# MoonLab-YH/AOD_MEH_HUA

Hardware: AMD Instinct MI355X
Metric: images/sec train+HUA-score, RetinaNet-R50 VOC 512^2 (higher is better)
Workload: dtype bf16x3

## Files before the change

### aod_meh_hua_amd/_C.py

```python
import ctypes as C
import os

import torch

_HERE = os.path.dirname(os.path.abspath(__file__))
LIB_PATH = os.environ.get('AOD_HIP_LIB') or os.path.join(_HERE, 'lib', 'libaodhip.so')


class AodHipError(RuntimeError):
    pass


if not os.path.exists(LIB_PATH):
    raise ImportError(f'{LIB_PATH} is missing: run `python -m aod_meh_hua_amd.build` (hipcc, gfx950). '
                      'There is no CPU fallback for the MEH/HUA hot path.')
lib = C.CDLL(LIB_PATH)


class ConvSeg(C.Structure):
    _fields_ = [('B', C.c_int32), ('H', C.c_int32), ('W', C.c_int32), ('OH', C.c_int32), ('OW', C.c_int32),
                ('src_row0', C.c_int64), ('dst_row0', C.c_int64)]


class ConvDesc(C.Structure):
# ... 22 lines not shown
    'aod_bottleneck128x3_fwd': (C.c_int, [P, I32, I32, I32, P, P, P, P, P, P, P, P, P, P, P, P, P]),
    'aod_bottleneck128_fwd': (C.c_int, [P, I32, I32, I32, P, P, P, P, P, P, P, P, P, P, P, P, P]),
    'aod_frag_pack': (C.c_int, [P, I32, I32, P]),
    'aod_frag_pack_item_bytes': (C.c_int, []),
    'aod_bottleneck256f_fwd': (C.c_int, [P, I32, I32, I32, P, P, P, P, P, P, P, P, P, P, P, P, P]),
    'aod_bottleneck256f_bwd': (C.c_int, [P, I32, I32, I32, P, P, P, P, P, P, P, P, P, P, P, P, P]),
    'aod_bottleneck_bwd': (C.c_int, [I32, P, I32, I32, I32, P, P, P, P, P, P, P, P, P, P, P, P, P]),
    'aod_bottleneck256_fwd': (C.c_int, [P, I32, I32, I32, P, P, P, P, P, P, P, P, P, P, P, P, P]),
    'aod_conv2d': (C.c_int, [C.POINTER(ConvDesc), P, P, P, P, P, P, P, P, P, P, P]),
    'aod_conv2d_ws_bytes': (SZ, [C.POINTER(ConvDesc)]),
    'aod_conv2d_ws': (C.c_int, [C.POINTER(ConvDesc), P, P, P, P, P, P, P, P, P, P, P, SZ, P]),
    'aod_conv2d_plan': (C.c_int, [C.POINTER(ConvDesc), I32, C.c_uint, C.POINTER(ConvPlan)]),
    'aod_conv2d_grouped': (C.c_int, [C.POINTER(ConvDesc), I32, P, P, P, P, P, P, P]),
    'aod_conv2d_ws_map': (C.c_int, [C.POINTER(ConvDesc), P, P, P, P, P, P, P, P, P, P, P, SZ, P, P, P]),
    'aod_conv2d_grouped_map': (C.c_int, [C.POINTER(ConvDesc), I32, P, P, P, P, P, P, P, P, P]),
    'aod_halo_conv3x3_applies': (C.c_int, [C.POINTER(ConvDesc)]),
    'aod_halo_conv3x3': (C.c_int, [C.POINTER(ConvDesc), P, P, P, P, P, P, P]),
    'aod_conv2d_wgrad': (C.c_int, [C.POINTER(ConvDesc), P, P, P, P, P]),
    'aod_conv2d_wgrad_splits': (C.c_int, [C.POINTER(ConvDesc)]),
    'aod_conv2d_wgrad_slabs': (C.c_int, [C.POINTER(ConvDesc), P, P, P, I32, I64, P, P]),
    'aod_conv2d_wgrad_slabs_map': (C.c_int, [C.POINTER(ConvDesc), P, P, P, I32, I64, P, P, P]),
    'aod_conv2d_wgrad_group_plan': (C.c_int, [P, I32, P]),
    'aod_conv2d_wgrad_grouped': (C.c_int, [P, I32, P, P, P, P, P, P, P]),
    'aod_conv2d_wgrad_plan': (C.c_int, [P, I32, P, P, P]),
    'aod_conv2d_wgrad_grouped_map': (C.c_int, [P, I32, P, P, P, P, P, P, P, P]),
    'aod_unpack_wgrad_slabs_grouped': (C.c_int, [I32, P, P, P, P, P, P, P, P, P, P, P, P, P, P, P, P, P]),
    'aod_unpack_wgrad_slabs': (C.c_int, [P, I32, I64, P, I32, I32, I32, I32, I32, I32, P, P, P, P, P, P, P]),
    'aod_conv_row_table_bytes': (SZ, [C.POINTER(ConvDesc)]),
    'aod_conv_row_table': (C.c_int, [C.POINTER(ConvDesc), P, P]),
    'aod_pack_weight_fwd': (C.c_int, [P, P, I32, I32, I32, I32, I32, P]),
# ... 124 lines not shown
```

### aod_meh_hua_amd/csrc/conv.hip

```cpp
#include "common.h"
#include "pointwise.h"
#include "conv_x3p.h"

struct ConvGroup { const bf16_t* x; const bf16_t* w; void* y; const float* pre_shift; const bf16_t* mask; float* colsum; const unsigned char* omap; };
struct ConvKParams {
  const bf16_t* x;
  const bf16_t* w;
  void* y;
  const float* pre_scale;
  const float* pre_shift;
  const bf16_t* res;
  const bf16_t* mask;
  const float* post_scale;
  bf16_t* zraw;
  float* colsum;
  int C, N, K, R, S, stride, pad, dil, transposed, relu, out_f32;
  int nseg, M;
  int tiles_m, tiles_n;
  int ksplit;
  float* ws;
  int perm;
  int ngroups;
  int interleave;
  const unsigned char* omap;
// ... 13 lines not shown
#ifdef AOD_TILE_TIMING
__device__ unsigned long long* g_tile_stamps = nullptr;
extern "C" int aod_dbg_set_tile_stamps(void* buf) { return (int)hipMemcpyToSymbol(HIP_SYMBOL(g_tile_stamps), &buf, sizeof(buf)); }
#define TSTAMP(k) do { if (g_tile_stamps && threadIdx.x == 0) g_tile_stamps[(size_t)blockIdx.x * 16 + (k)] = wall_clock64(); } while (0)
#else
#define TSTAMP(k) do {} while (0)
#endif

__device__ __forceinline__ unsigned udiv_small(unsigned n, unsigned d) {
  unsigned q = (unsigned)((float)n * __builtin_amdgcn_rcpf((float)d));
  const int r = (int)(n - q * d);
  q = r < 0 ? q - 1 : ((unsigned)r >= d ? q + 1 : q);
  return q;
}

__device__ __forceinline__ int xcd_swizzle(int bid, int nwg) {
  const int q = nwg >> 3, r = nwg & 7, xcd = bid & 7, j = bid >> 3;
  return (xcd < r ? xcd * (q + 1) : r * (q + 1) + (xcd - r) * q) + j;
}

template <int BM, int BN, int NT, int OPS, bool GROUPED, int ST, bool X3>
__global__ __launch_bounds__(NT) __attribute__((amdgpu_waves_per_eu(BM >= 192 ? 2 : (NT == 512 ? 4 : 1), BM >= 192 ? 2 : (NT == 512 ? 4 : 8)))) void conv_igemm_kernel(const ConvKParams p) {
  static_assert(NT == 256 || NT == 512, "4 or 8 waves");
  static_assert(ST == 2 || (ST == 3 && NT == 256), "LDS stages: 2, or 3 for the 4-wave forms");
  static_assert(!X3 || NT == 256 || (NT == 512 && (BM == 256 || BM == 192 || BM == 128)), "X3: the 4-wave forms, the 8-wave 256 x 256 / 192 x 192 tiles and (A/B) the 8-wave 128 x 128 tile");
  constexpr int BK = 64;
  constexpr int CPR = BK / 8;
  constexpr int RPP = NT / CPR;
  constexpr int A_IT = BM / RPP, B_IT = BN / RPP;
  constexpr int ROWB = BK * 2;
  constexpr int A_BYTES = BM * ROWB, B_BYTES = BN * ROWB, STAGE = A_BYTES + B_BYTES;
  constexpr int WAVES_M = NT / 128;
  constexpr int WM = BM / WAVES_M, WN = BN / 2;
// ... 3 lines not shown
  constexpr int EBM = BM / EP;
  constexpr bool PREFETCH = EP == 1 && !X3;
  extern __shared__ __attribute__((aligned(16))) char smem[];

  const int t = threadIdx.x;
  TSTAMP(0);
  const int lane = t & 63, wave = t >> 6;
  const int wm = wave >> 1, wn = wave & 1;
  const int nwg = p.tiles_m * p.tiles_n;
  int wg;
  if (!p.perm) wg = xcd_swizzle(blockIdx.x, nwg * (GROUPED ? p.ngroups : p.ksplit));
  else if ((nwg & 31) == 0) {
    const int x = blockIdx.x & 7, j = blockIdx.x >> 3, q = j & 3, k = j >> 2, tq = nwg >> 2;
    wg = q * tq + x * (tq >> 3) + k;
  } else wg = blockIdx.x;
  const bool il = GROUPED && p.interleave;
  const int tile = il ? wg / p.ngroups : wg % nwg, zz = il ? wg % p.ngroups : wg / nwg;
  const int kz = GROUPED ? 0 : zz;
  const int gi = GROUPED ? zz : 0;
#define AOD_GSEL(f, dflt) (GROUPED ? (gi == 0 ? p.grp[0].f : (gi == 1 ? p.grp[1].f : (gi == 2 ? p.grp[2].f : p.grp[3].f))) : (dflt))
  const bf16_t* const g_x = AOD_GSEL(x, p.x);
  const bf16_t* const g_w = AOD_GSEL(w, p.w);
  const float* const g_shift = AOD_GSEL(pre_shift, p.pre_shift);
#define g_y AOD_GSEL(y, p.y)
#define g_mask AOD_GSEL(mask, p.mask)
#define g_colsum AOD_GSEL(colsum, p.colsum)
  const int tile_n = tile % p.tiles_n, tile_m = tile / p.tiles_n;
  const int m0 = tile_m * BM, n0 = tile_n * BN;
  if constexpr (X3 && (GROUPED || NT == 256)) {
    const unsigned char* const om = AOD_GSEL(omap, p.omap);
    if (om) {
      const int mend = m0 + BM < p.M ? m0 + BM : p.M;
// ... 839 lines not shown
    const char* ksplit_steps = getenv("AOD_KSPLIT_STEPS");
    const char* stagger = getenv("AOD_STAGGER");
    const char* x3_taps_inner = getenv("AOD_X3_TAPS_INNER");
    const char* dgrad_lattice = getenv("AOD_DGRAD_LATTICE");
    const char* dgrad_classes = getenv("AOD_DGRAD_CLASSES");
    const char* tile_want = getenv("AOD_TILE_WANT");
    const char* tile_256 = getenv("AOD_TILE_256");
    const char* x3_128_w8 = getenv("AOD_X3_128_W8");
    const char* x3_128_st3 = getenv("AOD_X3_128_ST3");
    const char* tile_w8 = getenv("AOD_TILE_W8");
    const char* ring3 = getenv("AOD_RING3");
  };
  static const Once& once() { static const Once k{}; return k; }

  enum Call { X3P_OVER_256, X3_TILE_192, X3P_GROUPED, X3P, X3P_PRE, X3P_BN, X3P_DGRAD, X3P_LATTICE, X3P_MIN_STEPS, X3P_PRE_MIN_STEPS, X3P_MIN_TILES,
              X3P_ROT, SPARSE_BWD, NCALL };
  const char* val[NCALL];
  unsigned seen = 0;
  const char* call(Call k) {
    static const char* const names[NCALL] = {"AOD_X3P_OVER_256", "AOD_X3_TILE_192", "AOD_X3P_GROUPED", "AOD_X3P", "AOD_X3P_PRE", "AOD_X3P_BN",
                                             "AOD_X3P_DGRAD", "AOD_X3P_LATTICE", "AOD_X3P_MIN_STEPS", "AOD_X3P_PRE_MIN_STEPS", "AOD_X3P_MIN_TILES",
                                             "AOD_X3P_ROT", "AOD_SPARSE_BWD"};
    if (!((seen >> k) & 1u)) { val[k] = getenv(names[k]); seen |= 1u << k; }
    return val[k];
  }
  bool is(Call k, char c) { const char* v = call(k); return v && v[0] == c; }
};
static bool knob_is(const char* v, char c) { return v && v[0] == c; }

static int xp_cus() {
  static int cus[64];
  int dev = 0;
  if (hipGetDevice(&dev) != hipSuccess || dev < 0 || dev > 63) return 256;
  if (!cus[dev]) {
    int n = 0;
    if (hipDeviceGetAttribute(&n, hipDeviceAttributeMultiprocessorCount, dev) != hipSuccess || n <= 0) n = 256;
    cus[dev] = n;
// ... 74 lines not shown
                       nullptr, colsum ? colsum[0] : nullptr, p);
  if (rc) return rc;
  AOD_CHECK_ARG(!p.perm, "conv_grouped: class-major stride-2 dgrad launches are not grouped");
  p.ngroups = ngroups;
  for (int g = 0; g < ngroups; ++g) {
    AOD_CHECK_ARG(src[g] && w_packed[g] && dst[g], "conv_grouped: null operand in group %d", g);
    p.grp[g].x = (const bf16_t*)src[g]; p.grp[g].w = (const bf16_t*)w_packed[g]; p.grp[g].y = dst[g];
    p.grp[g].pre_shift = pre_shift ? pre_shift[g] : nullptr;
    p.grp[g].mask = mask ? (const bf16_t*)mask[g] : nullptr;
    p.grp[g].colsum = colsum ? colsum[g] : nullptr;
  }
  return 0;
}

struct MapGeo { int nseg, M, R, S, pad, dil; int segH[8], segW[8], seg_mend[8]; };
__global__ __launch_bounds__(256) void row_map_dilate_kernel(const unsigned char* __restrict__ in, unsigned char* __restrict__ out, const MapGeo g) {
  const int b = (int)(blockIdx.x * 256 + threadIdx.x);
  if (b >= (g.M + 63) >> 6) return;
  const int r0 = b << 6, r1 = r0 + 63 < g.M ? r0 + 63 : g.M - 1;
  const int up = (g.R - 1) * g.dil - g.pad, dn = g.pad, lf = (g.S - 1) * g.dil - g.pad, rt = g.pad;
  int any = 0;
  for (int sg = 0; sg < g.nseg; ++sg) {
    const int s0 = sg ? g.seg_mend[sg - 1] : 0, s1 = g.seg_mend[sg];
    const int lo = (r0 > s0 ? r0 : s0) - s0, hi = (r1 < s1 - 1 ? r1 : s1 - 1) - s0;
    if (lo > hi) continue;
    const int W = g.segW[sg], hw = g.segH[sg] * W;
    int a = lo - up * W - lf, z = hi + dn * W + rt;
    const int qa = (lo / W - up) * W, qz = (hi / W + dn + 1) * W - 1;
    a = a > qa ? a : qa; z = z < qz ? z : qz;
    const int ia = (lo / hw) * hw, iz = (hi / hw + 1) * hw - 1;
    a = a > ia ? a : ia; z = z < iz ? z : iz;
    for (int k = (s0 + a) >> 6; k <= (s0 + z) >> 6; ++k) any |= in[k];
  }
  out[b] = any ? 1 : 0;
}

static int conv_map_setup(ConvKParams& p, int ngroups, const void* const* in_map, void* const* out_map, hipStream_t st) {
  const int ng = ngroups ? ngroups : 1;
  bool any = false;
  for (int g = 0; g < ng; ++g) {
    AOD_CHECK_ARG(!in_map[g] == !out_map[g], "conv (map): member %d needs both its incoming and its outgoing map, or neither", g);
    any = any || in_map[g];
  }
  if (!any || p.M == 0) return 0;
  AOD_CHECK_ARG(p.x3 && p.transposed && p.stride == 1 && !p.out_f32 && !p.perm && !p.up_w, "conv (map): row-activity maps exist for the x3 stride-1 dgrad with X-layout rows only");
  AOD_CHECK_ARG((p.R - 1) * p.dil >= p.pad && (p.S - 1) * p.dil >= p.pad, "conv (map): padding beyond the filter");
  MapGeo mg;
  memset(&mg, 0, sizeof(mg));
  mg.nseg = p.nseg; mg.M = p.M; mg.R = p.R; mg.S = p.S; mg.pad = p.pad; mg.dil = p.dil;
// ... 5 lines not shown
  }
  const int nblk = (p.M + 63) >> 6;
  ConvKnobs kn;
  const bool dense = kn.is(ConvKnobs::SPARSE_BWD, '0');
  for (int g = 0; g < ng; ++g) {
    if (!in_map[g]) continue;
    hipLaunchKernelGGL(row_map_dilate_kernel, dim3((nblk + 255) / 256), dim3(256), 0, st, (const unsigned char*)in_map[g], (unsigned char*)out_map[g], mg);
    AOD_LAUNCH_CHECK();
    const float* const shift = ngroups ? p.grp[g].pre_shift : p.pre_shift;
    float* const cs = ngroups ? p.grp[g].colsum : p.colsum;
    const bool skip_ok = !dense && !shift && !p.pre_scale && !p.res && !p.post_scale && !p.zraw && !(cs && aod_get_deterministic());
    if (!skip_ok) continue;
    if (ngroups) { p.grp[g].omap = (const unsigned char*)out_map[g]; p.interleave = 1; }
    else p.omap = (const unsigned char*)out_map[g];
  }
  return 0;
}

extern "C" size_t aod_conv2d_ws_bytes(const aod_conv_desc_t* desc) {
  ConvKParams p;
  memset(&p, 0, sizeof(p));
  if (!desc || fill_params(desc, p) != 0 || p.M == 0) return 0;
  const int ks = choose_ksplit(p);
  return ks > 1 ? (size_t)ks * p.M * p.N * 4 : 0;
}

static void pw_args(const ConvKParams& p, PwArgs& a) {
  const long long s0 = p.seg_src0[0], d0 = p.seg_dst0[0];
  a.x = p.x + s0 * p.C; a.w = p.w; a.y = reinterpret_cast<bf16_t*>(p.y) + d0 * p.N;
  a.pre_scale = p.pre_scale; a.pre_shift = p.pre_shift;
// ... 238 lines not shown
  if (p.M == 0) return 0;
  rc = conv_plan(p, ngroups, false, pl);
  if (rc) return rc;
  AOD_CHECK_ARG(!in_map == !out_map, "conv_grouped (map): incoming and outgoing maps come together");
  if (in_map) {
    rc = conv_map_setup(p, ngroups, in_map, out_map, (hipStream_t)stream);
    if (rc) return rc;
  }
  return conv_launch(pl, p, nullptr, 0, (hipStream_t)stream);
}

extern "C" int aod_conv2d_grouped(const aod_conv_desc_t* desc, int ngroups, const void* const* src, const void* const* w_packed,
                                  void* const* dst, const float* const* pre_shift, const void* const* mask, float* const* colsum,
                                  aod_stream_t stream) {
  return aod_conv2d_grouped_map(desc, ngroups, src, w_packed, dst, pre_shift, mask, colsum, nullptr, nullptr, stream);
}

extern "C" int aod_conv2d(const aod_conv_desc_t* desc, const void* src, const void* w_packed, void* dst,
                          const float* pre_scale, const float* pre_shift, const void* res, const void* mask,
                          const float* post_scale, void* zraw, float* colsum, aod_stream_t stream) {
  return aod_conv2d_ws(desc, src, w_packed, dst, pre_scale, pre_shift, res, mask, post_scale, zraw, colsum, nullptr, 0, stream);
}

extern "C" int aod_conv2d_plan(const aod_conv_desc_t* desc, int ngroups, unsigned operand_flags, aod_conv_plan_t* out) {
  AOD_CHECK_ARG(desc && out && ngroups >= 0 && ngroups <= 4, "conv_plan: null pointer or ngroups outside 0..4");
  static char operand[16];
  char* const dst = operand + 8;
  auto has = [&](unsigned f) { return (operand_flags & f) ? (void*)operand : nullptr; };
  void* const res = (operand_flags & AOD_CONV_RES_IS_DST) ? (void*)dst : has(AOD_CONV_HAS_RES);
  ConvKParams p;
// ... 1182 lines not shown
```

### aod_meh_hua_amd/functional.py

```python
import torch
from torch.autograd import Function

from . import hipops as ho
from .hipops import Seg


def as_rows(x):
    B, C, H, W = x.shape
    xr = x.permute(0, 2, 3, 1)
    if not xr.is_contiguous():
        xr = xr.contiguous()
    return xr.view(B * H * W, C)


def as_nchw(rows, B, H, W):
    return rows.view(B, H, W, rows.shape[1]).permute(0, 3, 1, 2)


def multi_rows(tensors):
    rows = [as_rows(t) for t in tensors]
    if len(rows) == 1:
        t = tensors[0]
        return rows[0], [Seg(t.shape[0], t.shape[2], t.shape[3], 0)]
    rb = rows[0].shape[1] * rows[0].element_size()
# ... 331 lines not shown

def _grad_slice(w, device):
    dst = getattr(w, '_aod_grad_view', None)
    if dst is not None and (w.__dict__.get('_aod_view_busy') or dst.device != device
                            or (w.grad is not None and w.grad.data_ptr() == dst.data_ptr())):
        dst = None
    if dst is not None:
        w._aod_view_busy = True
        dst = dst.detach()
    return dst


_S1_OF = {}
_ROW_MAPS = {}
MAP_LOG = None


def _map_of(dz):
    e = _ROW_MAPS.get(dz.data_ptr())
    return e[0] if e is not None and e[1].shape == dz.shape and e[1].dtype == dz.dtype and ho.sparse_bwd() else None


def _keep_map(dx, rmap):
    if rmap is not None:
        if MAP_LOG is not None:
            MAP_LOG.append((tuple(dx.shape), rmap))
        _WgradQueue.begin_pass()
        _ROW_MAPS[dx.data_ptr()] = (rmap, dx)


# ... 299 lines not shown
    @staticmethod
    def forward(ctx, meta, wA, bA, wB, bB, *xs):
        nl = len(xs) // 2
        O, I, R, S = wA.shape
        rows, segs = zip(multi_rows(xs[:nl]), multi_rows(xs[nl:]))
        assert segs[0] == segs[1] and wB.shape == wA.shape, 'paired tower convs need identical geometry'
        cin = rows[0].shape[1]
        pis = [PREP.get(w, None, cin, 0.0) for w in (wA, wB)]
        rows, wfs, shifts = list(rows), [pi.wf for pi in pis], [bA.detach(), bB.detach()]
        rider = meta.get('rider')
        if rider is not None:
            convL, xL = rider
            rows.append(xL)
            wfs.append(PREP.get(convL.weight, None, cin, 0.0).wf)
            shifts.append(convL.bias.detach())
        outs, y_segs = ho.conv2d_rows_grouped(rows, list(segs[0]), wfs, O, R, S, 1, meta['pad'], meta['dil'], pre_shifts=shifts, relu=True,
                                              alg=(I, O))
        if rider is not None:
            meta['rider_out'] = outs[2]
        ctx.meta, ctx.x_segs, ctx.y_segs, ctx.nl = meta, list(segs[0]), y_segs, nl
        ctx.save_for_backward(wA, wB, rows[0], rows[1], outs[0], outs[1])
        return tuple(as_nchw(o[s.row0:s.row0 + s.rows], s.B, s.H, s.W) for o in outs[:2] for s in y_segs)

    @staticmethod
    def backward(ctx, *gouts):
        wA, wB, xA, xB, yA, yB = ctx.saved_tensors
        meta, nl, y_segs, x_segs = ctx.meta, ctx.nl, ctx.y_segs, ctx.x_segs
        O, I, R, S = wA.shape
        dsegs, xd = dense_segs(y_segs), dense_segs(x_segs)
        dzs, gws, gbs = [], [], []
        for gi, (w, x_rows, a_rows) in enumerate(((wA, xA, yA), (wB, xB, yB))):
            g_rows = _grad_rows(gouts[gi * nl:(gi + 1) * nl], y_segs, ho.width(O), w.device)
# ... 24 lines not shown
            dxs = ho.conv2d_dgrad_rows_grouped(dzs, dsegs, xd, wds, I, R, S, 1, meta['pad'], meta['dil'],
                                               masks=[xA if fuse[0] else None, xB if fuse[1] else None], colsums=s1_in, alg=(I, O),
                                               in_maps=rmaps if any(m is not None for m in rmaps) else None)
            if any(m is not None for m in rmaps):
                dxs, omaps = dxs
                for dx, om in zip(dxs, omaps):
                    _keep_map(dx, om)
            for gi in range(2):
                if fuse[gi]:
                    in_slots[gi].masked, in_slots[gi].s1 = True, s1_in[gi]
                for i, s in enumerate(xd):
                    gxs[gi * nl + i] = as_nchw(dxs[gi][s.row0:s.row0 + s.rows], s.B, s.H, s.W)
        return (None, gws[0], gbs[0], gws[1], gbs[1]) + tuple(gxs)


def conv_pair_act(xsA, xsB, convA, convB, sole_consumer=False, rider=None):
    import os
    wA, wB = convA.weight, convB.weight
    x3_ok = not ho.X3 or (wA.shape[0] % 256 == 0 and wA.shape[1] % 32 == 0 and wA.shape[1] * wA.shape[2] * wA.shape[3] >= 1024)
    ok = (x3_ok and os.environ.get('AOD_GROUP_TOWERS', '1') != '0' and wA.shape == wB.shape and wA.shape[0] % 8 == 0
          and wA.shape[0] >= 128 and convA.bias is not None and convB.bias is not None and convA.stride[0] == convB.stride[0] == 1
          and convA.padding == convB.padding and convA.dilation == convB.dilation and len(xsA) == len(xsB)
          and all(a.shape == b.shape and a.dtype == torch.bfloat16 for a, b in zip(xsA, xsB)))
    if not ok:
        r = (conv_bn_act(list(xsA), wA, bias=convA.bias, pad=convA.padding[0], dil=convA.dilation[0], relu=True, sole_consumer=sole_consumer),
             conv_bn_act(list(xsB), wB, bias=convB.bias, pad=convB.padding[0], dil=convB.dilation[0], relu=True, sole_consumer=sole_consumer))
        return r if rider is None else r + (None,)
    meta = dict(pad=convA.padding[0], dil=convA.dilation[0], slot=[None, None], in_slot=[None, None])
    if rider is not None:
        cl = rider[0]
        if (cl.weight.shape == wA.shape and cl.bias is not None and cl.padding == convA.padding and cl.dilation == convA.dilation
                and cl.stride[0] == 1 and rider[1].dtype == torch.bfloat16):
            meta['rider'] = rider
    grad = torch.is_grad_enabled()
    if grad:
        meta['slot'] = [ActSlot(), ActSlot()]
        if sole_consumer and _FUSE_ACT:
            for gi, xl in enumerate((xsA, xsB)):
                slots = [getattr(x, '_aod_slot', None) for x in xl]
                if slots[0] is not None and all(sl is slots[0] for sl in slots) and all(x.requires_grad for x in xl):
                    meta['in_slot'][gi] = slots[0]
                    slots[0].res_ok = False
    outs = ConvPairFn.apply(meta, wA, convA.bias, wB, convB.bias, *xsA, *xsB)
    nl = len(xsA)
    ya, yb = list(outs[:nl]), list(outs[nl:])
    if grad:
        for gi, ys in enumerate((ya, yb)):
            for o in ys:
# ... 573 lines not shown
```

### aod_meh_hua_amd/hipops.py

```python
import ctypes as C
import os
from dataclasses import dataclass
from typing import List, Optional, Sequence

import torch

from . import _C
from ._C import ConvDesc, ConvSeg, call, lib, ptr, stream


X3 = False
DETERMINISTIC = False


def set_deterministic(on=True):
    global DETERMINISTIC
    rc = lib.aod_set_deterministic(1 if on else 0)
    if rc < 0:
        raise RuntimeError(lib.aod_last_error().decode())
    DETERMINISTIC = bool(on)


def xw(c):
    return 2 * ((c + 31) // 32 * 32)
# ... 154 lines not shown
    z = torch.empty(rows, N, dtype=torch.bfloat16, device=x_rows.device) if save_z else None
    d = make_desc(Cin, N, R, S, stride, pad, dil, src_segs, dst_segs, False, relu, out_f32)
    if R == 3 and not save_z and _halo_applies(d, N, pre_scale, res, mask, post_scale):
        _prof('fwd', d, lambda: call('aod_halo_conv3x3', C.byref(d), ptr(x_rows), ptr(w_packed), ptr(out), ptr(pre_shift), None, None, stream()), alg)
        return out, dst_segs
    if (X3 and R == 3 and out_f32 and N <= 48 and not save_z and pre_scale is None and res is None and mask is None and post_scale is None
            and os.environ.get('AOD_HALO_X3', '1') != '0' and lib.aod_halo_conv3x3_x3_applies(C.byref(d))):
        _prof('fwd', d, lambda: call('aod_halo_conv3x3_x3', C.byref(d), ptr(x_rows), ptr(w_packed), ptr(out), ptr(pre_shift), stream()), alg)
        return out, dst_segs
    ws, wsb = _splitk_ws(d, x_rows.device)
    _prof('fwd', d, lambda: call('aod_conv2d_ws', C.byref(d), ptr(x_rows), ptr(w_packed), ptr(out), ptr(pre_scale), ptr(pre_shift),
                                 ptr(res), ptr(mask), ptr(post_scale), ptr(z), None, ptr(ws), wsb, stream()), alg)
    return (out, dst_segs, z) if save_z else (out, dst_segs)


def conv2d_rows_grouped(xs, src_segs, ws, N, R, S, stride=1, pad=0, dil=1, *, pre_shifts=None, relu=False, outs=None, alg=None):
    G = len(xs)
    Cin = xs[0].shape[1]
    dst_segs = out_segs(src_segs, R, S, stride, pad, dil)
    rows = sum(s.rows for s in dst_segs)
    if outs is None:
        outs = [torch.empty(rows, width(N), dtype=torch.bfloat16, device=xs[0].device) for _ in range(G)]
    d = make_desc(Cin, N, R, S, stride, pad, dil, src_segs, dst_segs, False, relu, False)
    arr = lambda ts: (C.c_void_p * G)(*[(t.data_ptr() if t is not None else None) for t in ts])
    for t in list(xs) + list(ws) + list(outs):
        ptr(t)
    keep = [arr(xs), arr(ws), arr(outs), arr(pre_shifts) if pre_shifts is not None else None]
    if PROFILE is None:
        call('aod_conv2d_grouped', C.byref(d), G, keep[0], keep[1], keep[2], keep[3], None, None, stream())
    else:
        for _ in range(1):
            _prof('fwd', d, lambda: call('aod_conv2d_grouped', C.byref(d), G, keep[0], keep[1], keep[2], keep[3], None, None, stream()),
                  (alg[0] * G, alg[1]) if alg is not None else (Cin * G, N))
    return outs, dst_segs


def sparse_bwd():
    return X3 and not DETERMINISTIC and os.environ.get('AOD_SPARSE_BWD', '1') != '0'


def row_map(rows, device):
    return torch.empty((rows + 63) // 64, dtype=torch.uint8, device=device)


def _maps_apply(dz_segs, x_segs, stride, out_f32):
    r = 0
    for a, b in zip(dz_segs, x_segs):
        if (a.B, a.H, a.W) != (b.B, b.H, b.W) or a.row0 != r or b.row0 != r:
            return False
# ... 674 lines not shown
```

### aod_meh_hua_amd/models/dense_heads/L_anchor_head.py

```python
import torch

from ...core.anchor import build_anchor_generator
from ...core.bbox import build_assigner, build_bbox_coder, build_sampler
from ...core.utils import multi_apply
from ...mmcv_lite import BaseModule, Conv2d, force_fp32
from ..builder import HEADS, build_loss

_NO_SAMPLING = ['EDL_Loss', 'EDL_Loss_2', 'EDL_Loss_3', 'EDL_Loss_BCE', 'FocalLoss', 'GHMC', 'QualityFocalLoss', 'EDL_FocalLoss',
                'EDL_BetaFocalLoss', 'EDL_FocalLoss_Dummy', 'EDL_Softmax_FocalLoss', 'EDL_Softmax_FocalLoss_Dummy',
                'EDL_Softmax_SL_FocalLoss', 'SSL_EDL_Softmax_FocalLoss']


class PackedGT(tuple):

    def __len__(self):
        return int(self[1].shape[0])


def pack_gts(gt_bboxes, gt_labels, device):
    if isinstance(gt_bboxes, PackedGT):
        return tuple.__getitem__(gt_bboxes, 0), tuple.__getitem__(gt_bboxes, 1), tuple.__getitem__(gt_bboxes, 2)
    B = len(gt_bboxes)
    counts = [int(g.shape[0]) for g in gt_bboxes]
    gmax = max(max(counts), 1)
# ... 112 lines not shown
        from ... import hipops as ho
        a = self.assigner
        return ho.max_iou_assign(flat, valid, gts, counts, labs, float(a.pos_iou_thr), float(a.neg_iou_thr), float(a.min_pos_iou),
                                 bool(a.gt_max_assign_all), self.num_classes, tuple(self.bbox_coder.means), tuple(self.bbox_coder.stds),
                                 level_start=starts)

    @force_fp32(apply_to=('cls_scores', 'bbox_preds', 'd_scores'))
    def loss(self, cls_scores, bbox_preds, D_scores, gt_bboxes, gt_labels, img_metas, gt_bboxes_ignore=None, **kwargs):
        featmap_sizes = [tuple(f.shape[-2:]) for f in cls_scores]
        assert len(featmap_sizes) == self.anchor_generator.num_levels
        device = cls_scores[0].device
        want_fused = False
        if self._can_defer_avg:
            from ... import functional as AF
            want_fused = AF.LOSS_LEVELS
        labels_list, lw_list, bt_list, bw_list, num_pos, nla = self.get_targets_batch(featmap_sizes, img_metas, gt_bboxes, gt_labels, device,
                                                                                      raw_num_pos=True)
        assert not self.sampling
        fused = None
        if want_fused:
            fused = self.loss_all_levels(cls_scores, bbox_preds, labels_list, lw_list, bt_list, bw_list, num_pos=num_pos, **kwargs)
        num_total_samples = fused[2] if fused is not None else num_pos.clamp(min=1).sum().float()
        B = cls_scores[0].shape[0]
        mlvl = self.anchor_generator.grid_anchors(featmap_sizes, device)
        all_anchor_list = [a[None].expand(B, a.shape[0], 4) for a in mlvl]
        head_info = ['cls_scores', 'bbox_preds', 'all_anchor_list', 'labels_list', 'label_weights_list', 'bbox_targets_list',
                     'bbox_weights_list', 'num_total_samples']
        head_out = (head_info, cls_scores, bbox_preds, all_anchor_list, labels_list, lw_list, bt_list, bw_list, num_total_samples)
        if self._can_defer_avg and fused is None:
            kwargs = dict(kwargs, grad_arena=AF.GradArena([c.shape[0] * c.shape[2] * c.shape[3] for c in cls_scores]))
        if fused is None:
            outs = multi_apply(self.loss_single, cls_scores, bbox_preds, all_anchor_list, labels_list, lw_list, bt_list, bw_list,
# ... 65 lines not shown
```

### aod_meh_hua_amd/models/dense_heads/Lambda_L2.py

```python
import numpy as np
import torch
import torch.nn as nn

from ... import functional as AF
from ...core.utils import multi_apply
from ...mmcv_lite import Conv2d, ConvModule, force_fp32
from ..builder import HEADS
from .L_anchor_head import L_AnchorHead


@HEADS.register_module()
class Lambda_L2Net(L_AnchorHead):
    def __init__(self, num_classes, in_channels, stacked_convs=4, conv_cfg=None, norm_cfg=None,
                 anchor_generator=dict(type='AnchorGenerator', octave_base_scale=4, scales_per_octave=3, ratios=[0.5, 1.0, 2.0],
                                       strides=[8, 16, 32, 64, 128]),
                 init_cfg=dict(type='Normal', layer='Conv2d', std=0.01,
                               override=dict(type='Normal', name='retina_cls', std=0.01, bias_prob=0.01)), **kwargs):
        self.stacked_convs, self.conv_cfg, self.norm_cfg = stacked_convs, conv_cfg, norm_cfg
        self.isTrainD = False
        super().__init__(num_classes, in_channels, anchor_generator=anchor_generator, init_cfg=init_cfg, **kwargs)
        self.L_names = ['retina_L', 'L_convs']

    def _init_layers(self):
        self.relu = nn.ReLU(inplace=True)
        self.cls_convs, self.reg_convs, self.L_convs = nn.ModuleList(), nn.ModuleList(), nn.ModuleList()
        for i in range(self.stacked_convs):
            chn = self.in_channels if i == 0 else self.feat_channels
            for tower in (self.cls_convs, self.reg_convs, self.L_convs):
                tower.append(ConvModule(chn, self.feat_channels, 3, stride=1, padding=1, conv_cfg=self.conv_cfg, norm_cfg=self.norm_cfg))
        self.retina_cls = Conv2d(self.feat_channels, self.num_anchors * self.cls_out_channels, 3, padding=1)
        self.retina_reg = Conv2d(self.feat_channels, self.num_anchors * 4, 3, padding=1)
        self.retina_L = Conv2d(self.feat_channels, self.num_anchors, 3, padding=1)

    def forward_train(self, x, img_metas, gt_bboxes, gt_labels=None, gt_bboxes_ignore=None, proposal_cfg=None, **kwargs):
        outs = self.forward(x, **kwargs)
        loss_inputs = outs + (None, gt_bboxes, gt_labels, img_metas)
        return self.loss(*loss_inputs, gt_bboxes_ignore=gt_bboxes_ignore, **kwargs)

    def forward_train_L(self, prev_loss, head_out, x, **kwargs):
        L_scores = self.forward_L(x, head_out, **kwargs)
        return self.loss_L(L_scores, head_out, prev_loss, **kwargs)

    def forward(self, feats, **kwargs):
        feats = list(feats)
        cls_feat, reg_feat = (list(t) for t in zip(*[AF.fork(f, 2) for f in feats]))
        if len(self.cls_convs) == len(self.reg_convs) and all(m.with_activation for m in list(self.cls_convs) + list(self.reg_convs)):
            import os
            ride = (torch.is_grad_enabled() and self.training and os.environ.get('AOD_MEH_RIDER', '1') != '0'
                    and len(self.L_convs) == len(self.cls_convs) and all(m.with_activation for m in self.L_convs)
                    and feats[0].dtype == torch.bfloat16)
            self._L_pre = None
            L_rows, L_outs = (AF.multi_rows([f.detach() for f in feats])[0] if ride else None), []
            for i, (cc, rc) in enumerate(zip(self.cls_convs, self.reg_convs)):
                if L_rows is not None:
                    cls_feat, reg_feat, L_rows = AF.conv_pair_act(cls_feat, reg_feat, cc.conv, rc.conv, sole_consumer=i > 0,
                                                                  rider=(self.L_convs[i].conv, L_rows))
                    L_outs.append(L_rows)
                else:
                    cls_feat, reg_feat = AF.conv_pair_act(cls_feat, reg_feat, cc.conv, rc.conv, sole_consumer=i > 0)
            if ride and len(L_outs) == len(self.L_convs) and all(o is not None for o in L_outs):
                self._L_pre = (feats[0].data_ptr(), tuple(feats[0].shape), [m.conv.weight._version for m in self.L_convs], L_outs)
        else:
            for i, conv in enumerate(self.cls_convs):
                cls_feat = conv(cls_feat, sole_consumer=i > 0)
            for i, conv in enumerate(self.reg_convs):
                reg_feat = conv(reg_feat, sole_consumer=i > 0)
        return (self.retina_cls(cls_feat, out_f32=True, sole_consumer=len(self.cls_convs) > 0),
                self.retina_reg(reg_feat, out_f32=True, sole_consumer=len(self.reg_convs) > 0, sparse_grad=True))

    def forward_cls_dropout(self, feats):
        assert AF.mc_dropout_active() and not torch.is_grad_enabled()
# ... 135 lines not shown
```

### include/aod_hip.h

```cpp
#ifndef AOD_HIP_H
#define AOD_HIP_H
#include <stddef.h>
#include <stdint.h>

#ifdef __cplusplus
extern "C" {
#endif

typedef void* aod_stream_t;

const char* aod_last_error(void);
int aod_version(void);

typedef struct {
  int32_t B, H, W;
  int32_t OH, OW;
  int64_t src_row0;
  int64_t dst_row0;
} aod_conv_seg_t;

typedef struct {
  int32_t C, N;
  int32_t R, S;
  int32_t stride, pad, dil;
// ... 58 lines not shown
                           const float* s2, const float* b2, const void* w3f, const float* s3, const float* b3, void* y, void* t1, void* t2,
                           aod_stream_t stream);
int aod_bottleneck256f_bwd(const void* g, int B, int H, int W, const void* wd3f, const void* wd2f, const void* wd1f, const void* act_t2,
                           const void* act_t1, const void* act_x, void* gx, void* gt2, void* gt1, float* colsum_t2, float* colsum_t1,
                           float* colsum_x, aod_stream_t stream);

int aod_conv2d_grouped(const aod_conv_desc_t* desc, int ngroups, const void* const* src, const void* const* w_packed, void* const* dst,
                       const float* const* pre_shift, const void* const* mask, float* const* colsum, aod_stream_t stream);

int aod_conv2d_ws_map(const aod_conv_desc_t* desc, const void* src, const void* w_packed, void* dst, const float* pre_scale,
                      const float* pre_shift, const void* res, const void* mask, const float* post_scale, void* zraw, float* colsum,
                      void* workspace, size_t workspace_bytes, const void* in_map, void* out_map, aod_stream_t stream);
int aod_conv2d_grouped_map(const aod_conv_desc_t* desc, int ngroups, const void* const* src, const void* const* w_packed, void* const* dst,
                           const float* const* pre_shift, const void* const* mask, float* const* colsum, const void* const* in_map,
                           void* const* out_map, aod_stream_t stream);

int aod_conv2d_wgrad(const aod_conv_desc_t* desc, const void* x, const void* dz, float* dw_f32,
                     const void* row_table, aod_stream_t stream);
int aod_conv2d_wgrad_splits(const aod_conv_desc_t* desc);
int aod_conv2d_wgrad_slabs(const aod_conv_desc_t* desc, const void* x, const void* dz, float* slabs, int nslabs, int64_t slab_stride,
                           const void* row_table, aod_stream_t stream);
int aod_conv2d_wgrad_group_plan(const aod_conv_desc_t* const* descs, int n, int32_t* splits_out);
int aod_conv2d_wgrad_grouped(const aod_conv_desc_t* const* descs, int n, const void* const* x, const void* const* dz, float* const* slabs,
                             const int32_t* nslabs, const int64_t* slab_stride, const void* const* row_table, aod_stream_t stream);
int aod_conv2d_wgrad_grouped_map(const aod_conv_desc_t* const* descs, int n, const void* const* x, const void* const* dz, float* const* slabs,
                                 const int32_t* nslabs, const int64_t* slab_stride, const void* const* row_table, const void* const* dz_map,
                                 aod_stream_t stream);
int aod_conv2d_wgrad_plan(const aod_conv_desc_t* const* descs, int n, int32_t* form, int32_t* splits, int32_t* rows_per_split);
int aod_conv2d_wgrad_slabs_map(const aod_conv_desc_t* desc, const void* x, const void* dz, float* slabs, int nslabs, int64_t slab_stride,
                               const void* row_table, const void* dz_map, aod_stream_t stream);
// ... 270 lines not shown
```

Baseline: 687.2.

## Skip forward reg-branch conv rows where bbox weights are zero via row-activity maps

Computes targets before the head forward, builds per-64-row activity maps from nonzero bbox weights, and dilates them back through the conv chain in one single-block kernel. The grouped forward conv launches then pass these maps as output maps for the reg and rider members, so tiles whose rows feed no regression loss can be skipped. The grouped tile/group dealing is also changed to rotate groups across XCDs when mapped. This adds two extra small kernels plus a host-side target computation moved earlier, and relies on skipped rows never being read downstream.

```diff
diff --git a/aod_meh_hua_amd/_C.py b/aod_meh_hua_amd/_C.py
--- a/aod_meh_hua_amd/_C.py
+++ b/aod_meh_hua_amd/_C.py
@@ -60,6 +60,9 @@
     'aod_conv2d_grouped': (C.c_int, [C.POINTER(ConvDesc), I32, P, P, P, P, P, P, P]),
     'aod_conv2d_ws_map': (C.c_int, [C.POINTER(ConvDesc), P, P, P, P, P, P, P, P, P, P, P, SZ, P, P, P]),
     'aod_conv2d_grouped_map': (C.c_int, [C.POINTER(ConvDesc), I32, P, P, P, P, P, P, P, P, P]),
+    'aod_fwd_row_maps': (C.c_int, [C.POINTER(ConvDesc), P, I32, I32, P, P]),
+    'aod_conv2d_grouped_fwd_map': (C.c_int, [C.POINTER(ConvDesc), I32, P, P, P, P, P, P]),
+    'aod_conv2d_grouped_deal': (C.c_int, [I32, I32, I32, P, P]),
     'aod_halo_conv3x3_applies': (C.c_int, [C.POINTER(ConvDesc)]),
     'aod_halo_conv3x3': (C.c_int, [C.POINTER(ConvDesc), P, P, P, P, P, P, P]),
     'aod_conv2d_wgrad': (C.c_int, [C.POINTER(ConvDesc), P, P, P, P, P]),
diff --git a/aod_meh_hua_amd/csrc/conv.hip b/aod_meh_hua_amd/csrc/conv.hip
--- a/aod_meh_hua_amd/csrc/conv.hip
+++ b/aod_meh_hua_amd/csrc/conv.hip
@@ -51,9 +51,20 @@
   return q;
 }
 
-__device__ __forceinline__ int xcd_swizzle(int bid, int nwg) {
+__host__ __device__ __forceinline__ int xcd_swizzle(int bid, int nwg) {
   const int q = nwg >> 3, r = nwg & 7, xcd = bid & 7, j = bid >> 3;
   return (xcd < r ? xcd * (q + 1) : r * (q + 1) + (xcd - r) * q) + j;
+}
+
+__host__ __device__ __forceinline__ void conv_grouped_deal(int bid, int nwg, int ngroups, int mapped, int& tile, int& group) {
+  if (!mapped) {
+    const int wg = xcd_swizzle(bid, nwg * ngroups);
+    tile = wg % nwg; group = wg / nwg;
+    return;
+  }
+  tile = bid / ngroups;
+  const int turn = (ngroups & 1) ? 0 : (tile * ngroups) >> 3;
+  group = (bid - tile * ngroups + turn) % ngroups;
 }
 
 template <int BM, int BN, int NT, int OPS, bool GROUPED, int ST, bool X3>
@@ -87,8 +98,8 @@
     const int x = blockIdx.x & 7, j = blockIdx.x >> 3, q = j & 3, k = j >> 2, tq = nwg >> 2;
     wg = q * tq + x * (tq >> 3) + k;
   } else wg = blockIdx.x;
-  const bool il = GROUPED && p.interleave;
-  const int tile = il ? wg / p.ngroups : wg % nwg, zz = il ? wg % p.ngroups : wg / nwg;
+  int tile = wg % nwg, zz = wg / nwg;
+  if (GROUPED && p.interleave) conv_grouped_deal(blockIdx.x, nwg, p.ngroups, 1, tile, zz);
   const int kz = GROUPED ? 0 : zz;
   const int gi = GROUPED ? zz : 0;
 #define AOD_GSEL(f, dflt) (GROUPED ? (gi == 0 ? p.grp[0].f : (gi == 1 ? p.grp[1].f : (gi == 2 ? p.grp[2].f : p.grp[3].f))) : (dflt))
@@ -958,13 +969,13 @@
   static const Once& once() { static const Once k{}; return k; }
 
   enum Call { X3P_OVER_256, X3_TILE_192, X3P_GROUPED, X3P, X3P_PRE, X3P_BN, X3P_DGRAD, X3P_LATTICE, X3P_MIN_STEPS, X3P_PRE_MIN_STEPS, X3P_MIN_TILES,
-              X3P_ROT, SPARSE_BWD, NCALL };
+              X3P_ROT, SPARSE_BWD, SPARSE_FWD, NCALL };
   const char* val[NCALL];
   unsigned seen = 0;
   const char* call(Call k) {
     static const char* const names[NCALL] = {"AOD_X3P_OVER_256", "AOD_X3_TILE_192", "AOD_X3P_GROUPED", "AOD_X3P", "AOD_X3P_PRE", "AOD_X3P_BN",
                                              "AOD_X3P_DGRAD", "AOD_X3P_LATTICE", "AOD_X3P_MIN_STEPS", "AOD_X3P_PRE_MIN_STEPS", "AOD_X3P_MIN_TILES",
-                                             "AOD_X3P_ROT", "AOD_SPARSE_BWD"};
+                                             "AOD_X3P_ROT", "AOD_SPARSE_BWD", "AOD_SPARSE_FWD"};
     if (!((seen >> k) & 1u)) { val[k] = getenv(names[k]); seen |= 1u << k; }
     return val[k];
   }
@@ -1069,9 +1080,7 @@
 }
 
 struct MapGeo { int nseg, M, R, S, pad, dil; int segH[8], segW[8], seg_mend[8]; };
-__global__ __launch_bounds__(256) void row_map_dilate_kernel(const unsigned char* __restrict__ in, unsigned char* __restrict__ out, const MapGeo g) {
-  const int b = (int)(blockIdx.x * 256 + threadIdx.x);
-  if (b >= (g.M + 63) >> 6) return;
+__device__ __forceinline__ unsigned char row_map_dilate_at(const unsigned char* in, int b, const MapGeo& g) {
   const int r0 = b << 6, r1 = r0 + 63 < g.M ? r0 + 63 : g.M - 1;
   const int up = (g.R - 1) * g.dil - g.pad, dn = g.pad, lf = (g.S - 1) * g.dil - g.pad, rt = g.pad;
   int any = 0;
@@ -1087,7 +1096,51 @@
     a = a > ia ? a : ia; z = z < iz ? z : iz;
     for (int k = (s0 + a) >> 6; k <= (s0 + z) >> 6; ++k) any |= in[k];
   }
-  out[b] = any ? 1 : 0;
+  return any ? 1 : 0;
+}
+__global__ __launch_bounds__(256) void row_map_dilate_kernel(const unsigned char* __restrict__ in, unsigned char* __restrict__ out, const MapGeo g) {
+  const int b = (int)(blockIdx.x * 256 + threadIdx.x);
+  if (b >= (g.M + 63) >> 6) return;
+  out[b] = row_map_dilate_at(in, b, g);
+}
+
+struct FwdMapChain { unsigned char* m[8]; int n; };
+__global__ __launch_bounds__(256) void fwd_row_map_kernel(const float* __restrict__ bw, unsigned char* __restrict__ out, long long rows, int fpr) {
+  const long long r0 = (long long)blockIdx.x * 64, r1 = r0 + 64 < rows ? r0 + 64 : rows;
+  const float4* const src = reinterpret_cast<const float4*>(bw + r0 * fpr);
+  const int n4 = (int)((r1 - r0) * (fpr >> 2));
+  int any = 0;
+  for (int i = (int)threadIdx.x; i < n4; i += 256) {
+    const float4 v = src[i];
+    any |= (v.x != 0.f || v.y != 0.f || v.z != 0.f || v.w != 0.f) ? 1 : 0;
+  }
+  any = __syncthreads_or(any);
+  if (threadIdx.x == 0) out[blockIdx.x] = any ? 1 : 0;
+}
+template <int LDS_BLOCKS>
+__global__ __launch_bounds__(1024) void fwd_map_chain_kernel(const FwdMapChain c, const MapGeo g) {
+  const int nblk = (g.M + 63) >> 6;
+  if constexpr (LDS_BLOCKS > 0) {
+    __shared__ unsigned char buf[2][LDS_BLOCKS];
+    for (int b = (int)threadIdx.x; b < nblk; b += 1024) buf[0][b] = c.m[0][b];
+    __syncthreads();
+    for (int k = 1; k < c.n; ++k) {
+      const unsigned char* const in = buf[(k - 1) & 1];
+      unsigned char* const out = buf[k & 1];
+      for (int b = (int)threadIdx.x; b < nblk; b += 1024) {
+        const unsigned char v = row_map_dilate_at(in, b, g);
+        out[b] = v;
+        c.m[k][b] = v;
+      }
+      __syncthreads();
+    }
+  } else {
+    for (int k = 1; k < c.n; ++k) {
+      for (int b = (int)threadIdx.x; b < nblk; b += 1024) c.m[k][b] = row_map_dilate_at(c.m[k - 1], b, g);
+      __threadfence_block();
+      __syncthreads();
+    }
+  }
 }
 
 static int conv_map_setup(ConvKParams& p, int ngroups, const void* const* in_map, void* const* out_map, hipStream_t st) {
@@ -1123,6 +1176,38 @@
     if (ngroups) { p.grp[g].omap = (const unsigned char*)out_map[g]; p.interleave = 1; }
     else p.omap = (const unsigned char*)out_map[g];
   }
+  return 0;
+}
+
+static int conv_map_geo(const ConvKParams& p, MapGeo& mg, bool dense_src) {
+  AOD_CHECK_ARG(p.x3 && p.stride == 1 && !p.out_f32 && !p.perm && !p.up_w, "conv (map): row-activity maps exist for x3 stride-1 launches with X-layout rows only");
+  AOD_CHECK_ARG((p.R - 1) * p.dil >= p.pad && (p.S - 1) * p.dil >= p.pad, "conv (map): padding beyond the filter");
+  memset(&mg, 0, sizeof(mg));
+  mg.nseg = p.nseg; mg.M = p.M; mg.R = p.R; mg.S = p.S; mg.pad = p.pad; mg.dil = p.dil;
+  for (int i = 0; i < p.nseg; ++i) {
+    const long long m0 = i ? p.seg_mend[i - 1] : 0;
+    AOD_CHECK_ARG(p.segH[i] == p.segOH[i] && p.segW[i] == p.segOW[i] && (!dense_src || p.seg_src0[i] == m0) && p.seg_dst0[i] == m0,
+                  "conv (map): segment %d is not a dense same-size map (the destination rows must be the GEMM rows)", i);
+    mg.segH[i] = p.segH[i]; mg.segW[i] = p.segW[i]; mg.seg_mend[i] = p.seg_mend[i];
+  }
+  return 0;
+}
+
+static int conv_fwd_map_setup(ConvKParams& p, int ngroups, const void* const* omap) {
+  bool any = false;
+  for (int g = 0; g < ngroups; ++g) any = any || omap[g];
+  if (!any || p.M == 0) return 0;
+  AOD_CHECK_ARG(!p.transposed, "conv_grouped (forward map): a dgrad descriptor -- its maps go through aod_conv2d_grouped_map");
+  AOD_CHECK_ARG(!p.pre_scale && !p.res && !p.post_scale && !p.zraw, "conv_grouped (forward map): scale / residual / raw-sum operands are not supported");
+  for (int g = 0; g < ngroups; ++g)
+    AOD_CHECK_ARG(!p.grp[g].mask && !p.grp[g].colsum, "conv_grouped (forward map): member %d carries a mask or column sums", g);
+  MapGeo mg;
+  const int rc = conv_map_geo(p, mg, false);
+  if (rc) return rc;
+  ConvKnobs kn;
+  if (kn.is(ConvKnobs::SPARSE_FWD, '0')) return 0;
+  for (int g = 0; g < ngroups; ++g) p.grp[g].omap = (const unsigned char*)omap[g];
+  p.interleave = 1;
   return 0;
 }
 
@@ -1391,6 +1476,63 @@
                                   void* const* dst, const float* const* pre_shift, const void* const* mask, float* const* colsum,
                                   aod_stream_t stream) {
   return aod_conv2d_grouped_map(desc, ngroups, src, w_packed, dst, pre_shift, mask, colsum, nullptr, nullptr, stream);
+}
+
+extern "C" int aod_conv2d_grouped_fwd_map(const aod_conv_desc_t* desc, int ngroups, const void* const* src, const void* const* w_packed,
+                                          void* const* dst, const float* const* pre_shift, const void* const* omap, aod_stream_t stream) {
+  ConvKParams p;
+  ConvPlan pl;
+  int rc = conv_params_grouped(desc, ngroups, src, w_packed, dst, pre_shift, nullptr, nullptr, p);
+  if (rc) return rc;
+  if (p.M == 0) return 0;
+  rc = conv_plan(p, ngroups, false, pl);
+  if (rc) return rc;
+  if (omap && pl.kind == AOD_CONV_PLAN_IGEMM && pl.x3) {
+    rc = conv_fwd_map_setup(p, ngroups, omap);
+    if (rc) return rc;
+  }
+  return conv_launch(pl, p, nullptr, 0, (hipStream_t)stream);
+}
+
+extern "C" int aod_fwd_row_maps(const aod_conv_desc_t* desc, const float* bbox_weights, int anchors, int nmaps, void* const* maps,
+                                aod_stream_t stream) {
+  AOD_CHECK_ARG(desc && bbox_weights && maps && anchors >= 1 && nmaps >= 1 && nmaps <= 8, "fwd_row_maps: null argument, or nmaps %d outside 1 .. 8", nmaps);
+  ConvKParams p;
+  memset(&p, 0, sizeof(p));
+  int rc = fill_params(desc, p);
+  if (rc) return rc;
+  AOD_CHECK_ARG(!p.transposed, "fwd_row_maps: a forward descriptor is expected");
+  MapGeo mg;
+  rc = conv_map_geo(p, mg, true);
+  if (rc) return rc;
+  if (p.M == 0) return 0;
+  FwdMapChain c;
+  memset(&c, 0, sizeof(c));
+  c.n = nmaps;
+  for (int k = 0; k < nmaps; ++k) {
+    AOD_CHECK_ARG(maps[k], "fwd_row_maps: map %d is null", k);
+    c.m[k] = (unsigned char*)maps[k];
+  }
+  AOD_CHECK_ARG(((uintptr_t)bbox_weights & 15) == 0, "fwd_row_maps: bbox_weights must be 16-byte aligned");
+  hipLaunchKernelGGL(fwd_row_map_kernel, dim3((p.M + 63) >> 6), dim3(256), 0, (hipStream_t)stream, bbox_weights, c.m[0], (long long)p.M, 4 * anchors);
+  AOD_LAUNCH_CHECK();
+  if (nmaps > 1) {
+    constexpr int LB = 16384;
+    if (((p.M + 63) >> 6) <= LB) hipLaunchKernelGGL(fwd_map_chain_kernel<LB>, dim3(1), dim3(1024), 0, (hipStream_t)stream, c, mg);
+    else hipLaunchKernelGGL(fwd_map_chain_kernel<0>, dim3(1), dim3(1024), 0, (hipStream_t)stream, c, mg);
+    AOD_LAUNCH_CHECK();
+  }
+  return 0;
+}
+
+extern "C" int aod_conv2d_grouped_deal(int nwg, int ngroups, int mapped, int32_t* tile, int32_t* group) {
+  AOD_CHECK_ARG(nwg >= 1 && ngroups >= 1 && ngroups <= 4 && tile && group, "conv_grouped_deal: nwg %d, ngroups %d", nwg, ngroups);
+  for (int b = 0; b < nwg * ngroups; ++b) {
+    int t, g;
+    conv_grouped_deal(b, nwg, ngroups, mapped ? 1 : 0, t, g);
+    tile[b] = t; group[b] = g;
+  }
+  return 0;
 }
 
 extern "C" int aod_conv2d(const aod_conv_desc_t* desc, const void* src, const void* w_packed, void* dst,
diff --git a/aod_meh_hua_amd/functional.py b/aod_meh_hua_amd/functional.py
--- a/aod_meh_hua_amd/functional.py
+++ b/aod_meh_hua_amd/functional.py
@@ -369,6 +369,7 @@
 _S1_OF = {}
 _ROW_MAPS = {}
 MAP_LOG = None
+FWD_MAP_LOG = None
 
 
 def _map_of(dz):
@@ -698,8 +699,12 @@
             rows.append(xL)
             wfs.append(PREP.get(convL.weight, None, cin, 0.0).wf)
             shifts.append(convL.bias.detach())
+        fmap = meta.get('fwd_map')
+        omaps = [None, fmap] + ([fmap] if rider is not None else []) if fmap is not None else None
+        if FWD_MAP_LOG is not None:
+            FWD_MAP_LOG.append((len(rows), (sum(s.rows for s in segs[0]), ho.width(O)), omaps))
         outs, y_segs = ho.conv2d_rows_grouped(rows, list(segs[0]), wfs, O, R, S, 1, meta['pad'], meta['dil'], pre_shifts=shifts, relu=True,
-                                              alg=(I, O))
+                                              alg=(I, O), omaps=omaps)
         if rider is not None:
             meta['rider_out'] = outs[2]
         ctx.meta, ctx.x_segs, ctx.y_segs, ctx.nl = meta, list(segs[0]), y_segs, nl
@@ -754,7 +759,7 @@
         return (None, gws[0], gbs[0], gws[1], gbs[1]) + tuple(gxs)
 
 
-def conv_pair_act(xsA, xsB, convA, convB, sole_consumer=False, rider=None):
+def conv_pair_act(xsA, xsB, convA, convB, sole_consumer=False, rider=None, fwd_map=None):
     import os
     wA, wB = convA.weight, convB.weight
     x3_ok = not ho.X3 or (wA.shape[0] % 256 == 0 and wA.shape[1] % 32 == 0 and wA.shape[1] * wA.shape[2] * wA.shape[3] >= 1024)
@@ -772,6 +777,8 @@
         if (cl.weight.shape == wA.shape and cl.bias is not None and cl.padding == convA.padding and cl.dilation == convA.dilation
                 and cl.stride[0] == 1 and rider[1].dtype == torch.bfloat16):
             meta['rider'] = rider
+    if fwd_map is not None and ho.sparse_fwd() and 'rider' in meta and convA.stride[0] == 1 and torch.is_grad_enabled():
+        meta['fwd_map'] = fwd_map
     grad = torch.is_grad_enabled()
     if grad:
         meta['slot'] = [ActSlot(), ActSlot()]
diff --git a/aod_meh_hua_amd/hipops.py b/aod_meh_hua_amd/hipops.py
--- a/aod_meh_hua_amd/hipops.py
+++ b/aod_meh_hua_amd/hipops.py
@@ -192,7 +192,7 @@
     return (out, dst_segs, z) if save_z else (out, dst_segs)
 
 
-def conv2d_rows_grouped(xs, src_segs, ws, N, R, S, stride=1, pad=0, dil=1, *, pre_shifts=None, relu=False, outs=None, alg=None):
+def conv2d_rows_grouped(xs, src_segs, ws, N, R, S, stride=1, pad=0, dil=1, *, pre_shifts=None, relu=False, outs=None, alg=None, omaps=None):
     G = len(xs)
     Cin = xs[0].shape[1]
     dst_segs = out_segs(src_segs, R, S, stride, pad, dil)
@@ -204,13 +204,35 @@
     for t in list(xs) + list(ws) + list(outs):
         ptr(t)
     keep = [arr(xs), arr(ws), arr(outs), arr(pre_shifts) if pre_shifts is not None else None]
+    if omaps is not None and any(m is not None for m in omaps):
+        assert (len(omaps) == G and X3 and stride == 1 and all((a.B, a.H, a.W) == (b.B, b.H, b.W) for a, b in zip(src_segs, dst_segs))), \
+            'forward maps: x3 stride-1 launches between same-size maps'
+        for m in omaps:
+            assert m is None or (m.dtype == torch.uint8 and m.is_cuda and m.numel() == (rows + 63) // 64)
+        keep.append(arr(omaps))
+        fn = lambda: call('aod_conv2d_grouped_fwd_map', C.byref(d), G, keep[0], keep[1], keep[2], keep[3], keep[4], stream())
+    else:
+        fn = lambda: call('aod_conv2d_grouped', C.byref(d), G, keep[0], keep[1], keep[2], keep[3], None, None, stream())
     if PROFILE is None:
-        call('aod_conv2d_grouped', C.byref(d), G, keep[0], keep[1], keep[2], keep[3], None, None, stream())
+        fn()
     else:
-        for _ in range(1):
-            _prof('fwd', d, lambda: call('aod_conv2d_grouped', C.byref(d), G, keep[0], keep[1], keep[2], keep[3], None, None, stream()),
-                  (alg[0] * G, alg[1]) if alg is not None else (Cin * G, N))
+        _prof('fwd', d, fn, (alg[0] * G, alg[1]) if alg is not None else (Cin * G, N))
     return outs, dst_segs
+
+
+def sparse_fwd():
+    return X3
+
+
+def fwd_row_maps(bbox_weights, segs, anchors, Cin, N, R, S, pad, dil, nmaps):
+    rows = sum(s.rows for s in segs)
+    assert bbox_weights.dtype == torch.float32 and bbox_weights.is_contiguous() and bbox_weights.numel() == rows * anchors * 4
+    d = make_desc(Cin, N, R, S, 1, pad, dil, segs, segs, False, True, False)
+    buf = torch.empty(nmaps, (rows + 63) // 64, dtype=torch.uint8, device=bbox_weights.device)
+    maps = list(buf.unbind(0))
+    keep = (C.c_void_p * nmaps)(*[m.data_ptr() for m in maps])
+    call('aod_fwd_row_maps', C.byref(d), ptr(bbox_weights), anchors, nmaps, keep, stream())
+    return maps
 
 
 def sparse_bwd():
diff --git a/aod_meh_hua_amd/models/dense_heads/L_anchor_head.py b/aod_meh_hua_amd/models/dense_heads/L_anchor_head.py
--- a/aod_meh_hua_amd/models/dense_heads/L_anchor_head.py
+++ b/aod_meh_hua_amd/models/dense_heads/L_anchor_head.py
@@ -150,8 +150,10 @@
         if self._can_defer_avg:
             from ... import functional as AF
             want_fused = AF.LOSS_LEVELS
-        labels_list, lw_list, bt_list, bw_list, num_pos, nla = self.get_targets_batch(featmap_sizes, img_metas, gt_bboxes, gt_labels, device,
-                                                                                      raw_num_pos=True)
+        targets = kwargs.pop('targets', None)
+        if targets is None:
+            targets = self.get_targets_batch(featmap_sizes, img_metas, gt_bboxes, gt_labels, device, raw_num_pos=True)
+        labels_list, lw_list, bt_list, bw_list, num_pos, nla = targets
         assert not self.sampling
         fused = None
         if want_fused:
diff --git a/aod_meh_hua_amd/models/dense_heads/Lambda_L2.py b/aod_meh_hua_amd/models/dense_heads/Lambda_L2.py
--- a/aod_meh_hua_amd/models/dense_heads/Lambda_L2.py
+++ b/aod_meh_hua_amd/models/dense_heads/Lambda_L2.py
@@ -33,28 +33,59 @@
         self.retina_L = Conv2d(self.feat_channels, self.num_anchors, 3, padding=1)
 
     def forward_train(self, x, img_metas, gt_bboxes, gt_labels=None, gt_bboxes_ignore=None, proposal_cfg=None, **kwargs):
-        outs = self.forward(x, **kwargs)
+        prepare = getattr(self, '_sparse_fwd_prepare', None)
+        targets, fwd_maps = prepare(x, img_metas, gt_bboxes, gt_labels, **kwargs) if prepare is not None else (None, None)
+        outs = self.forward(x, **kwargs) if fwd_maps is None else self.forward(x, fwd_maps=fwd_maps, **kwargs)
         loss_inputs = outs + (None, gt_bboxes, gt_labels, img_metas)
+        if targets is not None:
+            kwargs = dict(kwargs, targets=targets)
         return self.loss(*loss_inputs, gt_bboxes_ignore=gt_bboxes_ignore, **kwargs)
+
+    def _sparse_fwd_prepare(self, x, img_metas, gt_bboxes, gt_labels, **kwargs):
+        from ... import hipops as ho
+        x = list(x)
+        n = len(self.reg_convs)
+        ok = (ho.sparse_fwd() and torch.is_grad_enabled() and self.training and kwargs.get('Labeled', True) and not kwargs.get('Pseudo', False)
+              and type(self.loss_bbox).__name__ == 'L1Loss' and self._meh_form in ('l2', 'l1', 'msle') and self._rides(x)
+              and 1 <= n == len(self.cls_convs) <= 7 and all(m.with_activation for m in list(self.cls_convs) + list(self.reg_convs))
+              and all(m.conv.weight.shape[2:] == (3, 3) and m.conv.padding == (1, 1) and m.conv.dilation == (1, 1) and m.conv.stride == (1, 1)
+                      for m in list(self.reg_convs) + list(self.L_convs))
+              and self.retina_reg.weight.shape[2:] == (3, 3) and self.retina_L.weight.shape[2:] == (3, 3))
+        if not ok:
+            return None, None
+        featmap_sizes = [tuple(f.shape[-2:]) for f in x]
+        targets = self.get_targets_batch(featmap_sizes, img_metas, gt_bboxes, gt_labels, x[0].device, raw_num_pos=True)
+        bw = AF.dense_concat([t.reshape(-1, 4) for t in targets[3]])
+        if bw is None or bw.dtype != torch.float32:
+            return targets, None
+        B = x[0].shape[0]
+        segs = AF.dense_segs([ho.Seg(B, h, w, 0) for h, w in featmap_sizes])
+        c = self.feat_channels
+        return targets, ho.fwd_row_maps(bw, segs, self.num_anchors, ho.width(c), c, 3, 3, 1, 1, n + 1)
+
+    def _rides(self, feats):
+        import os
+        return (torch.is_grad_enabled() and self.training and os.environ.get('AOD_MEH_RIDER', '1') != '0'
+                and len(self.L_convs) == len(self.cls_convs) and all(m.with_activation for m in self.L_convs)
+                and feats[0].dtype == torch.bfloat16)
 
     def forward_train_L(self, prev_loss, head_out, x, **kwargs):
         L_scores = self.forward_L(x, head_out, **kwargs)
         return self.loss_L(L_scores, head_out, prev_loss, **kwargs)
 
-    def forward(self, feats, **kwargs):
+    def forward(self, feats, fwd_maps=None, **kwargs):
         feats = list(feats)
         cls_feat, reg_feat = (list(t) for t in zip(*[AF.fork(f, 2) for f in feats]))
         if len(self.cls_convs) == len(self.reg_convs) and all(m.with_activation for m in list(self.cls_convs) + list(self.reg_convs)):
-            import os
-            ride = (torch.is_grad_enabled() and self.training and os.environ.get('AOD_MEH_RIDER', '1') != '0'
-                    and len(self.L_convs) == len(self.cls_convs) and all(m.with_activation for m in self.L_convs)
-                    and feats[0].dtype == torch.bfloat16)
+            ride = self._rides(feats)
+            nl = len(self.cls_convs)
             self._L_pre = None
             L_rows, L_outs = (AF.multi_rows([f.detach() for f in feats])[0] if ride else None), []
             for i, (cc, rc) in enumerate(zip(self.cls_convs, self.reg_convs)):
                 if L_rows is not None:
                     cls_feat, reg_feat, L_rows = AF.conv_pair_act(cls_feat, reg_feat, cc.conv, rc.conv, sole_consumer=i > 0,
-                                                                  rider=(self.L_convs[i].conv, L_rows))
+                                                                  rider=(self.L_convs[i].conv, L_rows),
+                                                                  fwd_map=fwd_maps[nl - i] if fwd_maps is not None else None)
                     L_outs.append(L_rows)
                 else:
                     cls_feat, reg_feat = AF.conv_pair_act(cls_feat, reg_feat, cc.conv, rc.conv, sole_consumer=i > 0)
diff --git a/include/aod_hip.h b/include/aod_hip.h
--- a/include/aod_hip.h
+++ b/include/aod_hip.h
@@ -96,6 +96,11 @@
 int aod_conv2d_grouped_map(const aod_conv_desc_t* desc, int ngroups, const void* const* src, const void* const* w_packed, void* const* dst,
                            const float* const* pre_shift, const void* const* mask, float* const* colsum, const void* const* in_map,
                            void* const* out_map, aod_stream_t stream);
+
+int aod_fwd_row_maps(const aod_conv_desc_t* desc, const float* bbox_weights, int anchors, int nmaps, void* const* maps, aod_stream_t stream);
+int aod_conv2d_grouped_fwd_map(const aod_conv_desc_t* desc, int ngroups, const void* const* src, const void* const* w_packed, void* const* dst,
+                               const float* const* pre_shift, const void* const* omap, aod_stream_t stream);
+int aod_conv2d_grouped_deal(int nwg, int ngroups, int mapped, int32_t* tile, int32_t* group);
 
 int aod_conv2d_wgrad(const aod_conv_desc_t* desc, const void* x, const void* dz, float* dw_f32,
                      const void* row_table, aod_stream_t stream);
```

Result: faster. 737.9, median of 6 (+7.4%).
